# Damo12320/OptixPathtracer

Hardware: AMD Instinct MI355X
Metric: Msamples/sec at 1920x1080, max-depth 8; MSE vs reference (higher is better)
Workload: dtype f32; 1 GPU; BASELINE configs[1]: Diffuse sphere-in-box 1920x1080, 1024 spp, depth 8, 1xMI355X; scene=sphere_box_diffuse, triangles=34570, width=1920, height=1080, max_depth=8, material_mode=lambert, kernel=auto (wavefront), frames_per_launch=128, wavefront_streams=1, parallelism=spp-shard x1, batch_frames=128, queue_bytes=55207544320, queue_budget_bytes=77305217024, bvh_builder=auto (GPU binned SAH + GPU SAH-optimal BVH4 collapse), primary_dedup=True

## Files before the change

### include/ptamd.h

```cpp
#ifndef PTAMD_H
#define PTAMD_H
#include <stddef.h>
#include <stdint.h>

#ifdef __cplusplus
extern "C" {
#endif

#define PT_OK 0
#define PT_ERR_INVALID (-1)
#define PT_ERR_HIP (-2)
#define PT_ERR_STATE (-3)
#define PT_ERR_NOMEM (-4)

#define PT_MAT_DEFAULT 0
#define PT_MAT_LAMBERT 1
#define PT_MAT_CONDUCTOR 2
#define PT_MAT_DIELECTRIC 3
#define PT_MAT_LAYERED 4

#define PT_KERNEL_MEGA 0
#define PT_KERNEL_WAVEFRONT 1
#define PT_BVH_AUTO 0
#define PT_BVH_LBVH 1
// ... 85 lines not shown
    uint64_t pair_kernel_launches;
    uint64_t pair_kernel_rays;
    uint64_t pair_kernel_bytes;
    uint64_t pair_kernel_shadow_rays;
    uint64_t nee_unoccluded;
    uint64_t queue_bytes;
    uint64_t queue_budget;
    int32_t last_streams;
    int32_t last_batch_frames;
    uint64_t look_ahead_held;
    uint64_t lit_table_answers;
    uint64_t lit_table_cells;
    uint64_t lit_table_bits_set;
    uint64_t lit_table_bytes;
    double lit_table_build_ms;
    uint64_t geometry_commits;
    uint64_t geometry_refits;
    uint64_t geometry_rebuilds;
    double geometry_commit_ms;
    double bvh_sah_cost;
    double bvh_sah_cost_built;
} pt_stats;

typedef struct pt_renderer pt_renderer;

int pt_create(const pt_scene* scene, const pt_options* options, pt_renderer** out);
int pt_destroy(pt_renderer* r);

int pt_resize(pt_renderer* r, int32_t width, int32_t height);
int pt_set_camera(pt_renderer* r, const float position[3], const float inverse_view[16],
// ... 11 lines not shown
int pt_set_primary_dedup(pt_renderer* r, int32_t enable);
int pt_set_wavefront_streams(pt_renderer* r, int32_t streams);
int pt_set_band_split(pt_renderer* r, int32_t enable);
int pt_set_lit_table(pt_renderer* r, int32_t enable);
typedef struct pt_lit_table_info {
    int32_t active;
    int32_t lights;
    uint32_t triangles;
    uint32_t cells;
    uint32_t words_per_light;
    float delta;
    float margin;
} pt_lit_table_info;
int pt_lit_table_download(pt_renderer* r, pt_lit_table_info* info, uint32_t* tri_words, int64_t tri_bytes,
                          uint32_t* bits, int64_t bits_bytes);

typedef struct pt_launch_params {
    struct {
        float* color_buffer;
        int32_t size[2];
        uint32_t id;
    } frame;
    struct {
        float position[3];
        float inverse_view_matrix[16];
        float inverse_projection_matrix[16];
    } camera;
    const pt_point_light* point_lights;
    int32_t point_light_count;
    int32_t max_bounces;
// ... 87 lines not shown
```

### optixpathtracer_amd/capi.py

```python
from __future__ import annotations

import ctypes as C
import os
from pathlib import Path

_HERE = Path(__file__).resolve().parent
LIB_PATH = _HERE / "libptamd.so"

PT_MAT_DEFAULT, PT_MAT_LAMBERT, PT_MAT_CONDUCTOR, PT_MAT_DIELECTRIC, PT_MAT_LAYERED = range(5)
PT_KERNEL_MEGA, PT_KERNEL_WAVEFRONT, PT_KERNEL_AUTO = 0, 1, 2
PT_BVH_AUTO, PT_BVH_LBVH, PT_BVH_SAH, PT_BVH_PLOC, PT_BVH_SAH_GPU = 0, 1, 2, 3, 4
PT_GEOM_REFIT, PT_GEOM_REBUILD = 0, 1
PT_OK, PT_ERR_INVALID, PT_ERR_HIP, PT_ERR_STATE, PT_ERR_NOMEM = 0, -1, -2, -3, -4

MATERIAL_MODES = {
    "default": PT_MAT_DEFAULT,
    "lambert": PT_MAT_LAMBERT,
    "conductor": PT_MAT_CONDUCTOR,
    "dielectric": PT_MAT_DIELECTRIC,
    "layered": PT_MAT_LAYERED,
}


class PTError(RuntimeError):
# ... 104 lines not shown
        ("pair_kernel_launches", C.c_uint64),
        ("pair_kernel_rays", C.c_uint64),
        ("pair_kernel_bytes", C.c_uint64),
        ("pair_kernel_shadow_rays", C.c_uint64),
        ("nee_unoccluded", C.c_uint64),
        ("queue_bytes", C.c_uint64),
        ("queue_budget", C.c_uint64),
        ("last_streams", C.c_int32),
        ("last_batch_frames", C.c_int32),
        ("look_ahead_held", C.c_uint64),
        ("lit_table_answers", C.c_uint64),
        ("lit_table_cells", C.c_uint64),
        ("lit_table_bits_set", C.c_uint64),
        ("lit_table_bytes", C.c_uint64),
        ("lit_table_build_ms", C.c_double),
        ("geometry_commits", C.c_uint64),
        ("geometry_refits", C.c_uint64),
        ("geometry_rebuilds", C.c_uint64),
        ("geometry_commit_ms", C.c_double),
        ("bvh_sah_cost", C.c_double),
        ("bvh_sah_cost_built", C.c_double),
    ]


class pt_lit_table_info(C.Structure):
    _fields_ = [("active", C.c_int32), ("lights", C.c_int32), ("triangles", C.c_uint32), ("cells", C.c_uint32),
                ("words_per_light", C.c_uint32), ("delta", C.c_float), ("margin", C.c_float)]


class _pt_launch_frame(C.Structure):
# ... 35 lines not shown
    "pt_set_queue_budget": (C.c_int, [_R, C.c_int64]),
    "pt_get_trace_coherence": (C.c_int, [_R, C.POINTER(C.c_uint64)]),
    "pt_set_debug_hold": (C.c_int, [_R, C.c_int32]),
    "pt_set_traversal_stats": (C.c_int, [_R, C.c_int32]),
    "pt_set_kernel_timing": (C.c_int, [_R, C.c_int32]),
    "pt_render": (C.c_int, [_R, _FP]),
    "pt_launch": (C.c_int, [_R, C.POINTER(pt_launch_params)]),
    "pt_accum_clear": (C.c_int, [_R]),
    "pt_render_frames": (C.c_int, [_R, C.c_uint32, C.c_uint32]),
    "pt_set_primary_dedup": (C.c_int, [_R, C.c_int32]),
    "pt_set_band_split": (C.c_int, [_R, C.c_int32]),
    "pt_set_wavefront_streams": (C.c_int, [_R, C.c_int32]),
    "pt_set_lit_table": (C.c_int, [_R, C.c_int32]),
    "pt_lit_table_download": (C.c_int, [_R, C.POINTER(pt_lit_table_info), C.c_void_p, C.c_int64, C.c_void_p,
                                        C.c_int64]),
    "pt_render_accumulate": (C.c_int, [_R, C.c_uint32, C.c_uint32, _FP]),
    "pt_set_accum_device_buffer": (C.c_int, [_R, C.c_void_p]),
    "pt_accum_device_ptr": (C.c_void_p, [_R]),
    "pt_accum_download": (C.c_int, [_R, _FP, C.c_float]),
    "pt_set_accum_fp64": (C.c_int, [_R, C.c_int32]),
    "pt_accum_device_ptr64": (C.c_void_p, [_R]),
    "pt_accum_download64": (C.c_int, [_R, C.POINTER(C.c_double)]),
    "pt_synchronize": (C.c_int, [_R]),
    "pt_stream": (C.c_void_p, [_R]),
    "pt_device_count": (C.c_int32, [_R]),
    "pt_devices": (C.c_int, [_R, C.POINTER(C.c_int32), C.c_int32]),
    "pt_frame_id": (C.c_uint32, [_R]),
    "pt_set_frame_id": (C.c_int, [_R, C.c_uint32]),
    "pt_get_stats": (C.c_int, [_R, C.POINTER(pt_stats)]),
    "pt_stats_reset": (C.c_int, [_R]),
# ... 64 lines not shown
```

### optixpathtracer_amd/csrc/pt_capi.cpp

```cpp
#include <hip/hip_runtime.h>
#include <rccl/rccl.h>

#include <algorithm>
#include <cmath>
#include <cstdio>
#include <cstdlib>
#include <cstring>
#include <string>
#include <vector>

#include "../../include/ptamd.h"
#include "pt_internal.h"
#include "pt_lit.h"

using namespace pt;

namespace {

thread_local std::string g_last_error;

int fail(int code, const std::string& msg) {
    g_last_error = msg;
    return code;
}
// ... 38 lines not shown
            e = hipEventElapsedTime(&ms, start[i], stop[i]);
            *ms_sum += ms;
        }
        used = 0;
        return e;
    }
    void destroy() {
        for (hipEvent_t e : start) (void)hipEventDestroy(e);
        for (hipEvent_t e : stop) (void)hipEventDestroy(e);
        start.clear();
        stop.clear();
        used = 0;
    }
};

constexpr int kCounters = 28;
constexpr size_t kMaxPendingEvents = 4096;
constexpr int kMinTraversalStack = std::min(stack_capacity(PT_WF_STACK), stack_capacity(PT_MK_STACK));

struct GeomHost {
    std::vector<float4> verts, norms;
    std::vector<int4> tidx;
    std::vector<float> model;
    std::vector<int> voff;
    std::vector<int> has_normals, alpha;
    std::vector<float4> uvs;
    int n_meshes() const { return (int)has_normals.size(); }
    int normal_mode(int m) const {
        if (!has_normals[(size_t)m]) return 0;
        const float* M = &model[16 * (size_t)m];
        for (int r = 0; r < 3; ++r) {
// ... 216 lines not shown
    int lit_mode = -1;
    uint32_t* d_lit_tri = nullptr;
    uint32_t* d_lit_bits = nullptr;
    uint32_t lit_cells = 0, lit_words = 0;
    uint32_t lit_words_cap = 0;
    float lit_diag = 0.0f;
    uint32_t lit_version = 1, lit_built_version = 0;
    const void* lit_built_lights = nullptr;
    int lit_built_n = 0;
    bool lit_active = false;
    bool lit_launch_call = false;
    hipEvent_t lit_ev[2] = {nullptr, nullptr};
    bool lit_ev_pending = false;
    double lit_build_ms = 0.0;
    int64_t lit_bits_set = -1;

    DevScene scene() const {
        DevScene S;
        S.nodes = d_nodes;
        S.isect = d_isect;
        S.shade = d_shade;
        S.mats = d_mats;
        S.tuv = d_tuv;
        S.texels = d_texels;
        S.texinfo = d_texinfo;
        S.ntri = ntri;
        S.n_nodes = bvh_nodes;
        S.lds_nodes = nullptr;
        S.n_lds = 0;
        return S;
// ... 47 lines not shown
    L.lights = r->d_lights;
    L.n_lights = r->n_lights;
    L.max_bounces = r->max_bounces;
    L.frame_base = frame_base;
    L.n_frames = n_frames;
    L.accum = accum;
    L.accum64 = accum64;
    L.frame_stride = frame_stride;
    L.counters = r->d_counters;
    L.debug_pixel = r->d_debug ? r->debug_pixel : -1;
    L.debug_frame = r->debug_frame;
    L.debug = r->d_debug;
    L.lit_tri = r->lit_active ? r->d_lit_tri : nullptr;
    L.lit_bits = r->d_lit_bits;
    L.lit_words = r->lit_words;
    return L;
}

#ifndef PT_LIT_TABLE
#define PT_LIT_TABLE 1
#endif
bool lit_wanted(const pt_renderer* r) {
    const bool pays = r->material_mode == PT_MAT_LAMBERT || r->material_mode == PT_MAT_DEFAULT ||
                      r->material_mode == PT_MAT_LAYERED;
    const bool on = r->lit_mode < 0 ? PT_LIT_TABLE != 0 && pays && !r->lit_launch_call : r->lit_mode > 0;
    return on && r->d_lit_tri && r->d_lights && r->n_lights >= 1 && r->n_lights <= kLitMaxLights;
}
int lit_prepare(pt_renderer* r) {
    r->lit_active = lit_wanted(r);
    if (!r->lit_active) return PT_OK;
    if (r->lit_built_version == r->lit_version && r->lit_built_lights == r->d_lights && r->lit_built_n == r->n_lights)
        return PT_OK;
    if (!r->lit_ev[0]) {
        PT_HIP(hipEventCreate(&r->lit_ev[0]), "hipEventCreate");
        PT_HIP(hipEventCreate(&r->lit_ev[1]), "hipEventCreate");
    }
    PT_HIP(hipEventRecord(r->lit_ev[0], r->stream), "hipEventRecord");
    PT_HIP(lit_build(r->scene(), r->d_lit_tri, r->lit_cells, r->lit_words, r->d_lights, r->n_lights, r->d_lit_bits,
                     r->lit_diag, r->stream),
           "lit_build");
    PT_HIP(hipEventRecord(r->lit_ev[1], r->stream), "hipEventRecord");
    r->lit_ev_pending = true;
    r->lit_bits_set = -1;
    r->lit_built_version = r->lit_version;
    r->lit_built_lights = r->d_lights;
    r->lit_built_n = r->n_lights;
    return PT_OK;
}

size_t queue_bytes_held(const pt_renderer* r) {
    size_t b = r->wf.paths > 0 ? wavefront_bytes(r->wf.paths, r->wf.max_bounces) : 0;
    for (int k = 1; k < pt_renderer::kMaxWFStreams; ++k)
        if (r->xwf[k].paths > 0) b += wavefront_bytes(r->xwf[k].paths, r->xwf[k].max_bounces);
    return b;
}

size_t queue_budget_bytes(const pt_renderer* r) {
    if (r->queue_budget < 0) return SIZE_MAX;
    if (r->queue_budget > 0) return (size_t)r->queue_budget;
    size_t total = 0;
    if (hipDeviceTotalMem(&total, r->device) != hipSuccess || total == 0) {
        (void)hipGetLastError();
// ... 567 lines not shown
        e = hipMalloc(&r->d_lit_bits, sizeof(uint32_t) * (size_t)words * kLitMaxLights);
        if (e == hipSuccess) r->lit_words_cap = words;
    }
    if (e == hipSuccess && !r->d_lit_tri) e = hipMalloc(&r->d_lit_tri, sizeof(uint32_t) * ntri);
    if (e == hipSuccess)
        e = hipMemcpy(r->d_lit_tri, lit_words_host.data(), sizeof(uint32_t) * ntri, hipMemcpyHostToDevice);
    if (e != hipSuccess) {
        if (r->d_lit_tri) (void)hipFree(r->d_lit_tri);
        r->d_lit_tri = nullptr;
        r->lit_cells = r->lit_words = 0;
        return hip_fail(e, "lit table");
    }
    r->lit_cells = cells;
    r->lit_words = words;
    r->lit_diag = diag;
    return PT_OK;
}

}

extern "C" {

const char* pt_last_error(void) { return g_last_error.c_str(); }
const char* pt_version(void) { return "ptamd 0.1.0 gfx950"; }

int pt_create(const pt_scene* scene, const pt_options* options, pt_renderer** out) {
    if (!out) return fail(PT_ERR_INVALID, "pt_create: out is NULL");
    *out = nullptr;
    if (!scene || scene->n_meshes < 0 || (scene->n_meshes > 0 && !scene->meshes))
        return fail(PT_ERR_INVALID, "pt_create: invalid scene");
// ... 230 lines not shown
    (void)hipSetDevice(r->device);
    if (r->d_part) (void)hipFree(r->d_part);
    if (r->d_part64) (void)hipFree(r->d_part64);
    if (r->d_accum64) (void)hipFree(r->d_accum64);
    (void)hipSetDevice(r->device);
    if (r->d_nodes) (void)hipFree(r->d_nodes);
    if (r->d_isect) (void)hipFree(r->d_isect);
    if (r->d_shade) (void)hipFree(r->d_shade);
    if (r->d_mats) (void)hipFree(r->d_mats);
    if (r->d_tuv) (void)hipFree(r->d_tuv);
    if (r->d_texels) (void)hipFree(r->d_texels);
    if (r->d_texinfo) (void)hipFree(r->d_texinfo);
    if (r->d_lights) (void)hipFree(r->d_lights);
    if (r->d_lit_tri) (void)hipFree(r->d_lit_tri);
    if (r->d_lit_bits) (void)hipFree(r->d_lit_bits);
    if (r->d_overts) (void)hipFree(r->d_overts);
    if (r->d_onorms) (void)hipFree(r->d_onorms);
    if (r->d_tidx) (void)hipFree(r->d_tidx);
    if (r->d_rmesh) (void)hipFree(r->d_rmesh);
    if (r->d_sah_part) (void)hipFree(r->d_sah_part);
    for (hipEvent_t e : r->geom_ev)
        if (e) (void)hipEventDestroy(e);
    for (hipEvent_t e : r->lit_ev)
        if (e) (void)hipEventDestroy(e);
    if (r->d_frame) (void)hipFree(r->d_frame);
    ring_free(r);
    if (r->d_accum) (void)hipFree(r->d_accum);
    if (r->d_display) (void)hipFree(r->d_display);
    if (r->d_counters) (void)hipFree(r->d_counters);
    if (r->d_debug) (void)hipFree(r->d_debug);
    if (r->d_cancel_seen) (void)hipFree(r->d_cancel_seen);
    if (r->h_cancel) (void)hipHostFree(r->h_cancel);
    if (r->h_hold_release) (void)hipHostFree(r->h_hold_release);
    wavefront_free(r->wf);
    for (int k = 1; k < pt_renderer::kMaxWFStreams; ++k) {
        wavefront_free(r->xwf[k]);
        if (r->xstream[k]) (void)hipStreamDestroy(r->xstream[k]);
        if (r->ev_join[k]) (void)hipEventDestroy(r->ev_join[k]);
// ... 571 lines not shown
        r->lit_built_n == r->n_lights) {
        const size_t nw = (size_t)r->lit_words * (size_t)r->lit_built_n;
        if (r->lit_bits_set < 0) {
            std::vector<uint32_t> hb(nw);
            PT_HIP(hipMemcpy(hb.data(), r->d_lit_bits, sizeof(uint32_t) * nw, hipMemcpyDeviceToHost),
                   "download lit table");
            int64_t n = 0;
            for (uint32_t w : hb) n += __builtin_popcount(w);
            r->lit_bits_set = n;
        }
        out->lit_table_cells = r->lit_cells;
        out->lit_table_bits_set = (uint64_t)r->lit_bits_set;
        out->lit_table_bytes = sizeof(uint32_t) * ((size_t)r->ntri + (size_t)r->lit_words * kLitMaxLights);
        out->lit_table_build_ms = r->lit_build_ms;
    }
    out->geometry_commits = r->geom_commits;
    out->geometry_refits = r->geom_refits;
    out->geometry_rebuilds = r->geom_rebuilds;
    out->geometry_commit_ms = r->geom_commit_ms;
    out->bvh_sah_cost = r->sah_cost;
    out->bvh_sah_cost_built = r->sah_cost_built;
    for (pt_renderer* p : r->peers) {
        pt_stats ps;
        rc = pt_get_stats(p, &ps);
        if (rc) return rc;
        out->segments += ps.segments;
        out->samples += ps.samples;
        out->nodes_visited += ps.nodes_visited;
        out->tri_tests += ps.tri_tests;
        out->rays += ps.rays;
// ... 2 lines not shown
        out->wave_active_lanes += ps.wave_active_lanes;
        out->wave_node_steps += ps.wave_node_steps;
        out->wave_tri_steps += ps.wave_tri_steps;
        out->wave_refills += ps.wave_refills;
        out->lds_nodes_visited += ps.lds_nodes_visited;
        out->shade_kernel_items += ps.shade_kernel_items;
        out->shadow_rays += ps.shadow_rays;
        out->trace_kernel_rays += ps.trace_kernel_rays;
        out->trace_kernel_bytes += ps.trace_kernel_bytes;
        out->strict_retraces += ps.strict_retraces;
        out->nee_unoccluded += ps.nee_unoccluded;
        out->pair_kernel_rays += ps.pair_kernel_rays;
        out->pair_kernel_bytes += ps.pair_kernel_bytes;
        out->pair_kernel_shadow_rays += ps.pair_kernel_shadow_rays;
        out->lit_table_answers += ps.lit_table_answers;
        out->queue_bytes += ps.queue_bytes;
    }
    return PT_OK;
}

int pt_stats_reset(pt_renderer* r) {
    if (!r) return fail(PT_ERR_INVALID, "pt_stats_reset: NULL");
    int rc = pt_synchronize(r);
    if (rc) return rc;
    for (pt_renderer* p : r->peers) {
        if ((rc = pt_stats_reset(p)) != PT_OK) return rc;
    }
    PT_HIP(hipSetDevice(r->device), "hipSetDevice");
    PT_HIP(hipMemset(r->d_counters, 0, kCounters * sizeof(unsigned long long)), "hipMemset counters");
    r->samples = 0;
// ... 301 lines not shown
    info->margin = lit_margin(r->lit_diag);
    PT_HIP(hipStreamSynchronize(r->stream), "hipStreamSynchronize");
    if (tri_words) {
        if (tri_bytes != (int64_t)(sizeof(uint32_t) * (size_t)r->ntri))
            return fail(PT_ERR_INVALID, "pt_lit_table_download: tri_words size mismatch");
        PT_HIP(hipMemcpy(tri_words, r->d_lit_tri, (size_t)tri_bytes, hipMemcpyDeviceToHost), "download lit table");
    }
    if (bits) {
        if (bits_bytes != (int64_t)(sizeof(uint32_t) * (size_t)r->lit_words * (size_t)r->n_lights))
            return fail(PT_ERR_INVALID, "pt_lit_table_download: bits size mismatch");
        PT_HIP(hipMemcpy(bits, r->d_lit_bits, (size_t)bits_bytes, hipMemcpyDeviceToHost), "download lit table");
    }
    return PT_OK;
}

extern "C" int pt_set_band_split(pt_renderer* r, int32_t enable) {
    if (!r) return fail(PT_ERR_INVALID, "pt_set_band_split: NULL");
    int rc = collect_pending(r);
    if (rc) return rc;
    r->band_split = enable != 0;
    for (pt_renderer* p : r->peers) {
        if ((rc = pt_set_band_split(p, enable)) != PT_OK) return rc;
    }
    return PT_OK;
}

extern "C" int pt_set_kernel_timing(pt_renderer* r, int32_t enable) {
    if (!r) return fail(PT_ERR_INVALID, "pt_set_kernel_timing: NULL");
    int rc = collect_pending(r);
    if (rc) return rc;
// ... 7 lines not shown
```

### optixpathtracer_amd/csrc/pt_device.h

```cpp
#pragma once
#include "pt_bsdf.h"

namespace pt {

constexpr int kEmptyChild = (int)0x80000000;

struct __align__(16) BNode4 {
    float4 lox, hix, loy, hiy, loz, hiz;
    int4 child;
    int4 pad;
};

__device__ __forceinline__ int leaf_first(int c) { return (~c) >> 3; }
__device__ __forceinline__ int leaf_count(int c) { return ((~c) & 7) + 1; }

struct DevScene {
    const BNode4* nodes;
    const float4* isect;
    const float4* shade;
    const float4* mats;
    const float4* tuv;
    const uint32_t* texels;
    const int4* texinfo;
    int ntri;
// ... 19 lines not shown
    const DevLight* lights;
    int n_lights;
    int max_bounces;
    uint32_t frame_base;
    uint32_t n_frames;
    float* accum;
    double* accum64;
    size_t frame_stride;
    unsigned long long* counters;
    int debug_pixel;
    uint32_t debug_frame;
    float* debug;
    const uint32_t* lit_tri;
    const uint32_t* lit_bits;
    uint32_t lit_words;
};
constexpr int kDebugMaxBounces = 64;
constexpr int kDebugRecordFloats = 22;

__device__ __forceinline__ int debug_path_id(const DevLaunch& L) {
    const uint32_t f = L.debug_frame - L.frame_base;
    const int P = L.width * L.height, p = L.debug_pixel - L.width * L.row0;
    return (L.debug_pixel >= 0 && p >= 0 && p < P && f < L.n_frames) ? (int)f * P + p : -1;
}

struct Hit {
    float t, u, v;
    int tri;
    int orig;
    bool back;
// ... 758 lines not shown
```

### optixpathtracer_amd/csrc/pt_internal.h

```cpp
#pragma once
#include <hip/hip_runtime.h>

#include <algorithm>
#include <vector>

#include "pt_device.h"

namespace pt {

struct BuildInput {
    const float4* tri_orig;
    const float4* nrm_orig;
    const float4* uv_orig;
    int n;
    float cmin[3], cmax[3];
    int builder;
    const float4* tri_host;
};
constexpr int kBuilderPLOC = 0;
constexpr int kBuilderLBVH = 1;
constexpr int kBuilderSAH = 2;
constexpr int kBuilderSAHGPU = 3;

void sah_binary_tree(const float4* tri, int n, std::vector<uint32_t>& order, std::vector<int2>& child,
// ... 53 lines not shown
hipError_t launch_wavefront_frame(int mode, bool stats, const DevScene& S, const DevLaunch& L, const WFState& W,
                                  uint32_t frame, int nf, bool primary_dedup, int cus, hipStream_t stream,
                                  const hipEvent_t* trace_events,
                                  int* n_timed = nullptr, hipEvent_t accum_wait = nullptr,
                                  hipEvent_t accum_done = nullptr, const hipEvent_t* shade_events = nullptr,
                                  int* n_shade_timed = nullptr, bool wide_trace = false);

hipError_t launch_render(int kernel, int mode, bool stats, const DevScene& S, const DevLaunch& L,
                         hipStream_t stream);
hipError_t launch_trace(const DevScene& S, const float* d_rays, int n, int* d_prim, float* d_thit, float* d_u,
                        float* d_v, int* d_back, int any_hit, hipStream_t stream);

bool lit_subdivide(const float4* isect, int ntri, std::vector<uint32_t>& words, uint32_t* cells, float* diagonal);
hipError_t lit_build(const DevScene& S, const uint32_t* tri_words, uint32_t cells, uint32_t words,
                     const DevLight* lights, int n_lights, uint32_t* bits, float diag, hipStream_t stream);

struct RefitMesh {
    float m[16];
    int dirty;
    int normal_mode;
    int pad[2];
};
hipError_t refit_rebake(const RefitMesh* meshes, const float4* overts, const float4* onorms, const int4* tidx, int n,
                        float4* isect, float4* shade, hipStream_t stream);
hipError_t refit_levels(BNode4* nodes, const float4* isect, const std::vector<int>& level_base, hipStream_t stream);
int sah_partial_blocks(int n_nodes);
hipError_t sah_partial_launch(const BNode4* nodes, int n_nodes, double* partial, hipStream_t stream);

hipError_t display_fill(float* p, size_t n, float v, hipStream_t stream);
hipError_t display_blend(float* fb, const float* frame, size_t n, float w, bool continuous, hipStream_t stream);
// ... 3 lines not shown
```

### optixpathtracer_amd/csrc/pt_lit.hip

```cpp
#include "pt_internal.h"
#include "pt_lit.h"

namespace pt {

bool lit_subdivide(const float4* isect, int ntri, std::vector<uint32_t>& words, uint32_t* cells, float* diagonal) {
    words.clear();
    *cells = 0;
    *diagonal = 0.0f;
    if (ntri <= 0) return false;
    float lo[3] = {INFINITY, INFINITY, INFINITY}, hi[3] = {-INFINITY, -INFINITY, -INFINITY};
    for (int t = 0; t < ntri; ++t) {
        const float4 A = isect[3 * t], E1 = isect[3 * t + 1], E2 = isect[3 * t + 2];
        const float v[3][3] = {{A.x, A.y, A.z}, {A.x + E1.x, A.y + E1.y, A.z + E1.z}, {A.x + E2.x, A.y + E2.y, A.z + E2.z}};
        for (int k = 0; k < 3; ++k)
            for (int a = 0; a < 3; ++a) {
                if (!(fabsf(v[k][a]) <= kLitMaxCoord)) return false;
                lo[a] = std::min(lo[a], v[k][a]);
                hi[a] = std::max(hi[a], v[k][a]);
            }
    }
    const double dx = (double)hi[0] - lo[0], dy = (double)hi[1] - lo[1], dz = (double)hi[2] - lo[2];
    const float diag = (float)std::sqrt(dx * dx + dy * dy + dz * dz);
    if (!(diag > 0.0f)) return false;
    const float target = kLitCellFraction * diag;
// ... 72 lines not shown
        } else {
            const int first = leaf_first(c), cnt = leaf_count(c);
            for (int q = 0; q < cnt; ++q) {
                const int u = first + q;
                const float4 UA = S.isect[3 * u], U1 = S.isect[3 * u + 1], U2 = S.isect[3 * u + 2];
                const double pa[3] = {UA.x, UA.y, UA.z};
                const double pb[3] = {(double)UA.x + U1.x, (double)UA.y + U1.y, (double)UA.z + U1.z};
                const double pc[3] = {(double)UA.x + U2.x, (double)UA.y + U2.y, (double)UA.z + U2.z};
                if (!lit_tri_outside(P, pa, pb, pc)) return;
            }
        }
    }
    atomicOr(&bits[(size_t)li * words + (cell >> 5)], 1u << (cell & 31));
}

}

hipError_t lit_build(const DevScene& S, const uint32_t* tri_words, uint32_t cells, uint32_t words,
                     const DevLight* lights, int n_lights, uint32_t* bits, float diag, hipStream_t stream) {
    hipError_t e = hipMemsetAsync(bits, 0, sizeof(uint32_t) * (size_t)words * (size_t)n_lights, stream);
    if (e != hipSuccess || n_lights <= 0) return e;
    const uint64_t n = (uint64_t)cells * (uint64_t)n_lights;
    hipLaunchKernelGGL(k_lit_build, dim3((unsigned)((n + kLitBlock - 1) / kLitBlock)), dim3(kLitBlock), 0, stream, S,
                       tri_words, cells, words, lights, n_lights, bits, diag);
    return hipGetLastError();
}

}
```

### optixpathtracer_amd/csrc/pt_wavefront.hip

```cpp
#include <type_traits>
#include <unordered_map>

#include "pt_internal.h"
#include "pt_lit.h"

namespace pt {

namespace {

constexpr int kBlockWF = 256;
#ifndef PT_TRACE_BLOCK
#define PT_TRACE_BLOCK 256
#endif
constexpr int kBlockTrace = PT_TRACE_BLOCK;
constexpr int kStack = PT_WF_STACK;
#ifndef PT_LDS_NODES
#define PT_LDS_NODES 49
#endif
constexpr int kLdsNodes = PT_LDS_NODES;
#ifndef PT_TRACE_BLOCK_WIDE
#define PT_TRACE_BLOCK_WIDE 768
#endif
#ifndef PT_LDS_NODES_WIDE
#define PT_LDS_NODES_WIDE 150
// ... 635 lines not shown
    return next_bounce < max_bounces && length(beta) > 0.00001f;
}

__device__ __forceinline__ int lit_cell(const DevLaunch& L, const Hit& h) {
    const uint32_t w = L.lit_tri[h.tri];
    const int k = lit_level(w);
    return k == kLitNoCells ? -1 : (int)(lit_first(w) + lit_cell_index(k, h.u, h.v));
}
__device__ __forceinline__ bool lit_bit(const DevLaunch& L, int li, int cell) {
    return (L.lit_bits[(size_t)li * L.lit_words + ((uint32_t)cell >> 5)] >> (cell & 31)) & 1u;
}
__device__ __forceinline__ void lit_count_wave(bool answered, int* lds) {
    const unsigned long long m = __ballot(answered ? 1 : 0);
    if (lane_id() == 0) lds[threadIdx.x >> 6] = __popcll(m);
}
template <int WAVES>
__device__ __forceinline__ void lit_count_block(const DevLaunch& L, const int* lds) {
    if (threadIdx.x != 0 || !L.counters) return;
    int tot = 0;
    for (int w = 0; w < WAVES; ++w) tot += lds[w];
    if (tot > 0) atomicAdd(&L.counters[27], (unsigned long long)tot);
}

__device__ __forceinline__ int vis0_index(const DevLaunch& L, int path, int li) {
    const int P1 = L.width * L.height;
    return li * P1 + path % P1;
}

template <bool TEX>
__global__ __launch_bounds__(kBlockWF) void k_shadow0_setup(DevScene S, DevLaunch L, WFState W) {
    const int P1 = L.width * L.height;
    const int nl = L.n_lights;
    const int n = P1 * nl;
    if (wf_cancelled(W)) return;
    for (int k = blockIdx.x * blockDim.x + threadIdx.x; k < n; k += gridDim.x * blockDim.x) {
        const int li = k / P1, p = k - li * P1;
// ... 16 lines not shown
    if (blockIdx.x == 0 && threadIdx.x == 0) *cnt(W, 0, kShadowQ) = n;
}

template <int MODE, bool TEX, bool SHADE0>
__global__ __launch_bounds__(shf_block(MODE), shf_waves(MODE)) void k_shade_fused(DevScene S, DevLaunch L, WFState W, int b, int vis0) {
    constexpr bool shade0 = SHADE0;
    constexpr bool kBetaQ = MODE == kModeLambert;
    constexpr bool kShareOrigin = MODE == kModeLambert;
    constexpr int kBlock = shf_block(MODE), kWaves = kBlock / 64;
    const int n = *cnt(W, b, kQueue);
    const float4* rd = W.ray_d[b & 1];
    float4* no = W.ray_o[(b + 1) & 1];
    float4* nd = W.ray_d[(b + 1) & 1];
    __shared__ int lds_sh[kSortKeys * kWaves + kSortKeys + 1], lds_q[kSortKeys * kWaves + kSortKeys + 1];
    __shared__ int lds_lit[kWaves];
    const bool lit = !vis0 && L.lit_tri;
    if (blockIdx.x == 0 && threadIdx.x == 0 && L.counters) atomicAdd(&L.counters[15], (unsigned long long)n);
    if ((int)(blockIdx.x * kBlock) >= n) return;
    {
        const int i = (int)(blockIdx.x * kBlock + threadIdx.x);
        const bool valid = i < n && !wf_cancelled(W);
        bool emit_shadow = false, emit_next = false, lit_answer = false;
        f3 so, sdir, contrib, o, d, beta;
        uint32_t seed = 0;
        float stmax = 0.0f;
        int path = 0;
        int shadow_light = 0;
        const int P1 = L.width * L.height;
        float4 l0 = make_float4(0.0f, 0.0f, 0.0f, 0.0f);
        if (valid) {
            const float4 hv = ldqs(W.hit + i);
            const float4 c_q = shade0 ? make_float4(0.0f, 0.0f, 0.0f, 0.0f) : ldqs(rd + i);
            const float4 bv_q = (!shade0 && kBetaQ) ? ldqs(queue_beta(W, b) + i) : make_float4(0.0f, 0.0f, 0.0f, 0.0f);
            path = __float_as_int(hv.x);
            const Hit h = decode_hit(hv);
            if (h.tri >= 0) {
                const int lit_c = lit ? lit_cell(L, h) : -1;
                const float4 c = shade0 ? ldqs(rd + path % P1) : c_q;
                d = mk(c.x, c.y, c.z);
                SurfaceHit sf;
                reconstruct<TEX>(S, h, d, sf);
                if (shade0) {
// ... 25 lines not shown
                        f3 Li = mk(lt.cr, lt.cg, lt.cb) / d2;
                        contrib = ((beta * spectrum) * Li) / (P * 1.0f);
                        lit_answer = lit_c >= 0 && dot(ldir, sf.ng) > kLitDelta && lit_bit(L, li, lit_c);
                        if (vis0 || lit_answer) {
                            if (lit_answer || W.vis[vis0_index(L, path, li)]) {
                                const float4 l = shade0 ? l0 : W.L[path];
                                l0 = make_float4(l.x + contrib.x, l.y + contrib.y, l.z + contrib.z, 0.0f);
                                if (!shade0) W.L[path] = l0;
                            }
                        } else {
                            so = sf.pos + 1e-3f * sf.ng;
                            sdir = normalize(ldir);
                            stmax = length(ldir);
                            emit_shadow = true;
                            shadow_light = li;
                        }
                    }
                }
                BSample bs;
                if (b + 1 < L.max_bounces &&
                    bsdf_sample<MODE>(seed, sf.albedo, sf.roughness, conductor, sf.wo, bs)) {
                    emit_next = continue_path(sf, bs, beta, o, d, b + 1, L.max_bounces);
                    if (!kBetaQ) stqs(W.beta + path, make_float4(beta.x, beta.y, beta.z, __uint_as_float(seed)));
                }
            }
        }
        if (shade0 && valid) W.L[path] = l0;
        if (lit) lit_count_wave(lit_answer, lds_lit);
        const int qi = PT_SORT_EXT ? block_append_sorted<kWaves, kSortKeys>(cnt(W, b + 1, kQueue), emit_next ? octant(d) : -1, lds_q)
                                   : block_append<kWaves>(cnt(W, b + 1, kQueue), emit_next, lds_q);
        if (lit) lit_count_block<kWaves>(L, lds_lit);
        if (emit_next) {
            stqs(no + qi, make_float4(o.x, o.y, o.z, __int_as_float(path)));
            stqs(nd + qi, make_float4(d.x, d.y, d.z, 0.0f));
            if (kBetaQ) stqs(queue_beta(W, b + 1) + qi, make_float4(beta.x, beta.y, beta.z, __uint_as_float(seed)));
        }
        const int si = PT_SORT_SHADOW ? block_append_sorted<kWaves, kSortKeys>(cnt(W, b, kShadowQ),
                                                                              emit_shadow ? (shadow_light & (kSortKeys - 1)) : -1, lds_sh)
                                      : block_append<kWaves>(cnt(W, b, kShadowQ), emit_shadow, lds_sh);
        if (emit_shadow) {
            const bool share = kShareOrigin && emit_next;
            if (!share) stqs(W.sh_o + si, make_float4(so.x, so.y, so.z, __int_as_float(path)));
            stqs(W.sh_d + si, make_float4(sdir.x, sdir.y, sdir.z, stmax));
            stqs(W.sh_c + si, make_float4(contrib.x, contrib.y, contrib.z, __int_as_float(share ? qi : -1)));
        }
    }
}

template <int MODE, bool TEX>
__global__ __launch_bounds__(shf_block(MODE), 1) void k_shade0_pixel(DevScene S, DevLaunch L, WFState W, int nf) {
    constexpr bool kBetaQ = MODE == kModeLambert;
    constexpr int kBlock = shf_block(MODE), kWaves = kBlock / 64;
    const int P1 = L.width * L.height;
    __shared__ int lds_q[kSortKeys * kWaves + kSortKeys + 1];
// ... 155 lines not shown
        atomicAdd(&counters[6], (unsigned long long)(n_ext + n_sh));
        atomicAdd(&counters[7], 48ull * (unsigned long long)(n_ext + n_sh));
        atomicAdd(&counters[16], (unsigned long long)(n_ext + n_sh));
        atomicAdd(&counters[17], 48ull * (unsigned long long)(n_ext + n_sh));
        atomicAdd(&counters[19], (unsigned long long)n_sh);
    }
    flush_trav_stats<STATS>(counters, ts);
}

template <int MODE, bool TEX>
__global__ __launch_bounds__(kBlockShA) void k_shade_a(DevScene S, DevLaunch L, WFState W, int b, int vis0) {
    const int n = *cnt(W, b, kQueue);
    const float4* rd = W.ray_d[b & 1];
    __shared__ int lds_sh[kWavesShA + 1];
    __shared__ int lds_nee[kNeeBuckets * (kWavesShA + 1)], lds_smp[kSmpBuckets * (kWavesShA + 1)];
    __shared__ int lds_lit[kWavesShA];
    const bool lit = !vis0 && L.lit_tri;
    if ((int)(blockIdx.x * kBlockShA) >= n) return;
    const int i = (int)(blockIdx.x * kBlockShA + threadIdx.x);
    bool emit = false, lit_answer = false;
    int nee_bucket = -1, smp_bucket = -1, code = 0;
    f3 so, sdir;
    float stmax = 0.0f;
    if (i < n && !wf_cancelled(W)) {
        const float4 hv = W.hit[i];
        const float4 c = rd[i];
        const int path = __float_as_int(hv.x);
        const Hit h = decode_hit(hv);
        if (h.tri >= 0) {
            const int lit_c = lit ? lit_cell(L, h) : -1;
            SurfaceHit sf;
            reconstruct<TEX>(S, h, mk(c.x, c.y, c.z), sf);
            float4 bv = W.beta[path];
            uint32_t seed = __float_as_uint(bv.w);
            if (path == debug_path_id(L)) {
// ... 18 lines not shown
                f3 ldir = mk(lt.px, lt.py, lt.pz) - sf.pos;
                const f3 ln = normalize(ldir);
                int nb = 0;
                if (MODE == kModeLayered || !conductor)
                    nb = PT_NEE_CROSS && !same_hemisphere(sf.wo, to_local(sf.fr, ln)) ? kNeeCross
                                                                                     : nee_layered_bucket(bk, sf.albedo);
                lit_answer = lit_c >= 0 && dot(ldir, sf.ng) > kLitDelta && lit_bit(L, li, lit_c);
                if (vis0 || lit_answer) {
                    if (lit_answer || W.vis[vis0_index(L, path, li)]) nee_bucket = nb;
                } else {
                    so = sf.pos + 1e-3f * sf.ng;
                    sdir = ln;
                    stmax = length(ldir);
                    code = i | (nb << kItemBits);
                    emit = true;
                }
            }
        }
    }
    if (lit) lit_count_wave(lit_answer, lds_lit);
    const int si = block_append<kWavesShA>(cnt(W, b, kShadowQ), emit, lds_sh);
    if (lit) lit_count_block<kWavesShA>(L, lds_lit);
    if (emit) {
        W.sh_o[si] = make_float4(so.x, so.y, so.z, __int_as_float(code));
        W.sh_d[si] = make_float4(sdir.x, sdir.y, sdir.z, stmax);
    }
    const int ni = block_append_k<kWavesShA, kNeeBuckets>(cnt(W, b, kNee0), nee_bucket, lds_nee);
    if (nee_bucket >= 0) W.nq[nee_index(W, nee_bucket, ni)] = i;
    const int mi = block_append_k<kWavesShA, kSmpBuckets>(cnt(W, b, kSmp0), smp_bucket, lds_smp);
    if (smp_bucket >= 0) W.sq[smp_index(W, smp_bucket, mi)] = i;
}

template <bool TEX, int BLK = kBlockTrace>
__global__ __launch_bounds__(BLK, wf_waves(false)) void k_shadow_vis(DevScene S, WFState W, int b, int table,
                                                                      unsigned long long* counters) {
    const int n = *cnt(W, b, kShadowQ);
    if (blockIdx.x == 0 && threadIdx.x == 0 && counters) atomicAdd(&counters[5], (unsigned long long)n);
// ... 580 lines not shown
```

### optixpathtracer_amd/renderer.py

```python
from __future__ import annotations

import ctypes as C
import dataclasses

import numpy as np

from . import capi
from .capi import check, fptr, load
from .scenes import Scene


def _f32(a, shape=None) -> np.ndarray:
    a = np.ascontiguousarray(a, dtype=np.float32)
    if shape is not None:
        a = a.reshape(shape)
    return a


class _SceneBinding:

    def __init__(self, scene: Scene):
        self.keep = []
        meshes = (capi.pt_mesh * max(1, len(scene.meshes)))()
        for i, m in enumerate(scene.meshes):
# ... 222 lines not shown
    def set_lit_table(self, enable: bool | None) -> None:
        check(self.lib.pt_set_lit_table(self.h, -1 if enable is None else (1 if enable else 0)), "pt_set_lit_table")

    def lit_table(self):
        info = capi.pt_lit_table_info()
        check(self.lib.pt_lit_table_download(self.h, C.byref(info), None, 0, None, 0), "pt_lit_table_download")
        d = {k: getattr(info, k) for k, _ in capi.pt_lit_table_info._fields_}
        if not info.active:
            return d, None, None
        tri = np.zeros(info.triangles, np.uint32)
        bits = np.zeros((info.lights, info.words_per_light), np.uint32)
        check(self.lib.pt_lit_table_download(self.h, C.byref(info), tri.ctypes.data, tri.nbytes, bits.ctypes.data,
                                             bits.nbytes), "pt_lit_table_download")
        return d, tri, bits

    def render_accumulate(self, spp: int, first_frame_id: int = 1) -> np.ndarray:
        w, h = self.size
        out = np.empty((h, w, 3), np.float32)
        check(self.lib.pt_render_accumulate(self.h, int(spp), int(first_frame_id), fptr(out)),
              "pt_render_accumulate")
        return out

    def set_accum_device_buffer(self, ptr: int | None) -> None:
        check(self.lib.pt_set_accum_device_buffer(self.h, C.c_void_p(ptr) if ptr else None),
              "pt_set_accum_device_buffer")

    def accum(self, scale: float = 1.0) -> np.ndarray:
        w, h = self.size
        out = np.empty((h, w, 3), np.float32)
        check(self.lib.pt_accum_download(self.h, fptr(out), float(scale)), "pt_accum_download")
# ... 94 lines not shown
```

Measured before the change: 1701 Msamples/sec.

## Add per-cell occluder table to resolve shadow rays with one triangle test

Builds a per-light, per-surface-cell table on the GPU. Each entry records the triangle hit by a ray from the cell centre toward the light. During shading, a shadow ray for an unlit cell first tests that cached triangle, and if it blocks the ray, no shadow ray is queued or traced through the BVH. This cuts shadow-queue traffic and any-hit traversal, at the cost of a build kernel, extra memory, a table lookup per shading point, and a possible stats-path download.

```diff
diff --git a/include/ptamd.h b/include/ptamd.h
--- a/include/ptamd.h
+++ b/include/ptamd.h
@@ -123,6 +123,10 @@
     uint64_t lit_table_bits_set;
     uint64_t lit_table_bytes;
     double lit_table_build_ms;
+    uint64_t occluder_table_bytes;
+    uint64_t occluder_table_candidates;
+    double occluder_table_build_ms;
+    uint64_t occluder_table_answers;
     uint64_t geometry_commits;
     uint64_t geometry_refits;
     uint64_t geometry_rebuilds;
@@ -164,6 +168,9 @@
 } pt_lit_table_info;
 int pt_lit_table_download(pt_renderer* r, pt_lit_table_info* info, uint32_t* tri_words, int64_t tri_bytes,
                           uint32_t* bits, int64_t bits_bytes);
+int pt_set_occluder_table(pt_renderer* r, int32_t enable);
+int pt_occluder_table_download(pt_renderer* r, int64_t* entries_out, int32_t* entries, int64_t bytes);
+int pt_occluder_table_upload(pt_renderer* r, const int32_t* entries, int64_t bytes);
 
 typedef struct pt_launch_params {
     struct {
diff --git a/optixpathtracer_amd/capi.py b/optixpathtracer_amd/capi.py
--- a/optixpathtracer_amd/capi.py
+++ b/optixpathtracer_amd/capi.py
@@ -142,6 +142,10 @@
         ("lit_table_bits_set", C.c_uint64),
         ("lit_table_bytes", C.c_uint64),
         ("lit_table_build_ms", C.c_double),
+        ("occluder_table_bytes", C.c_uint64),
+        ("occluder_table_candidates", C.c_uint64),
+        ("occluder_table_build_ms", C.c_double),
+        ("occluder_table_answers", C.c_uint64),
         ("geometry_commits", C.c_uint64),
         ("geometry_refits", C.c_uint64),
         ("geometry_rebuilds", C.c_uint64),
@@ -207,6 +211,9 @@
     "pt_set_lit_table": (C.c_int, [_R, C.c_int32]),
     "pt_lit_table_download": (C.c_int, [_R, C.POINTER(pt_lit_table_info), C.c_void_p, C.c_int64, C.c_void_p,
                                         C.c_int64]),
+    "pt_set_occluder_table": (C.c_int, [_R, C.c_int32]),
+    "pt_occluder_table_download": (C.c_int, [_R, C.POINTER(C.c_int64), C.c_void_p, C.c_int64]),
+    "pt_occluder_table_upload": (C.c_int, [_R, C.c_void_p, C.c_int64]),
     "pt_render_accumulate": (C.c_int, [_R, C.c_uint32, C.c_uint32, _FP]),
     "pt_set_accum_device_buffer": (C.c_int, [_R, C.c_void_p]),
     "pt_accum_device_ptr": (C.c_void_p, [_R]),
diff --git a/optixpathtracer_amd/csrc/pt_capi.cpp b/optixpathtracer_amd/csrc/pt_capi.cpp
--- a/optixpathtracer_amd/csrc/pt_capi.cpp
+++ b/optixpathtracer_amd/csrc/pt_capi.cpp
@@ -76,7 +76,7 @@
     }
 };
 
-constexpr int kCounters = 28;
+constexpr int kCounters = 29;
 constexpr size_t kMaxPendingEvents = 4096;
 constexpr int kMinTraversalStack = std::min(stack_capacity(PT_WF_STACK), stack_capacity(PT_MK_STACK));
 
@@ -323,6 +323,18 @@
     bool lit_ev_pending = false;
     double lit_build_ms = 0.0;
     int64_t lit_bits_set = -1;
+    int occ_mode = -1;
+    int* d_occ = nullptr;
+    size_t occ_cap = 0;
+    bool occ_alloc_failed = false;
+    uint32_t occ_built_version = 0;
+    const void* occ_built_lights = nullptr;
+    int occ_built_n = 0;
+    bool occ_active = false;
+    hipEvent_t occ_ev[2] = {nullptr, nullptr};
+    bool occ_ev_pending = false;
+    double occ_build_ms = 0.0;
+    int64_t occ_candidates = -1;
 
     DevScene scene() const {
         DevScene S;
@@ -400,6 +412,8 @@
     L.lit_tri = r->lit_active ? r->d_lit_tri : nullptr;
     L.lit_bits = r->d_lit_bits;
     L.lit_words = r->lit_words;
+    L.occ_tab = r->lit_active && r->occ_active ? r->d_occ : nullptr;
+    L.lit_cells = r->lit_cells;
     return L;
 }
 
@@ -412,11 +426,57 @@
     const bool on = r->lit_mode < 0 ? PT_LIT_TABLE != 0 && pays && !r->lit_launch_call : r->lit_mode > 0;
     return on && r->d_lit_tri && r->d_lights && r->n_lights >= 1 && r->n_lights <= kLitMaxLights;
 }
+#ifndef PT_OCC_TABLE
+#define PT_OCC_TABLE 1
+#endif
+bool occ_wanted(const pt_renderer* r) {
+    const bool has_code = r->material_mode == PT_MAT_LAMBERT || r->material_mode == PT_MAT_DEFAULT ||
+                          r->material_mode == PT_MAT_LAYERED;
+    const bool pays = has_code;
+    const bool on = r->occ_mode < 0 ? PT_OCC_TABLE != 0 && pays && r->lit_mode < 0 : r->occ_mode > 0;
+    return on && has_code && !r->occ_alloc_failed && lit_wanted(r);
+}
+int occ_prepare(pt_renderer* r) {
+    r->occ_active = occ_wanted(r);
+    if (!r->occ_active) return PT_OK;
+    if (r->occ_built_version == r->lit_version && r->occ_built_lights == r->d_lights && r->occ_built_n == r->n_lights)
+        return PT_OK;
+    const size_t need = (size_t)r->lit_cells * (size_t)r->n_lights;
+    if (need > r->occ_cap) {
+        if (r->d_occ) (void)hipFree(r->d_occ);
+        r->d_occ = nullptr;
+        r->occ_cap = 0;
+        if (hipMalloc(&r->d_occ, sizeof(int) * need) != hipSuccess) {
+            (void)hipGetLastError();
+            r->d_occ = nullptr;
+            r->occ_alloc_failed = true;
+            r->occ_active = false;
+            return PT_OK;
+        }
+        r->occ_cap = need;
+    }
+    if (!r->occ_ev[0]) {
+        PT_HIP(hipEventCreate(&r->occ_ev[0]), "hipEventCreate");
+        PT_HIP(hipEventCreate(&r->occ_ev[1]), "hipEventCreate");
+    }
+    PT_HIP(hipEventRecord(r->occ_ev[0], r->stream), "hipEventRecord");
+    PT_HIP(occ_build(r->scene(), r->d_lit_tri, r->lit_cells, r->lit_words, r->d_lights, r->n_lights, r->d_lit_bits,
+                     r->d_occ, r->stream),
+           "occ_build");
+    PT_HIP(hipEventRecord(r->occ_ev[1], r->stream), "hipEventRecord");
+    r->occ_ev_pending = true;
+    r->occ_candidates = -1;
+    r->occ_built_version = r->lit_version;
+    r->occ_built_lights = r->d_lights;
+    r->occ_built_n = r->n_lights;
+    return PT_OK;
+}
 int lit_prepare(pt_renderer* r) {
     r->lit_active = lit_wanted(r);
+    r->occ_active = false;
     if (!r->lit_active) return PT_OK;
     if (r->lit_built_version == r->lit_version && r->lit_built_lights == r->d_lights && r->lit_built_n == r->n_lights)
-        return PT_OK;
+        return occ_prepare(r);
     if (!r->lit_ev[0]) {
         PT_HIP(hipEventCreate(&r->lit_ev[0]), "hipEventCreate");
         PT_HIP(hipEventCreate(&r->lit_ev[1]), "hipEventCreate");
@@ -431,7 +491,7 @@
     r->lit_built_version = r->lit_version;
     r->lit_built_lights = r->d_lights;
     r->lit_built_n = r->n_lights;
-    return PT_OK;
+    return occ_prepare(r);
 }
 
 size_t queue_bytes_held(const pt_renderer* r) {
@@ -1029,6 +1089,7 @@
     r->lit_cells = cells;
     r->lit_words = words;
     r->lit_diag = diag;
+    r->occ_alloc_failed = false;
     return PT_OK;
 }
 
@@ -1289,6 +1350,7 @@
     if (r->d_lights) (void)hipFree(r->d_lights);
     if (r->d_lit_tri) (void)hipFree(r->d_lit_tri);
     if (r->d_lit_bits) (void)hipFree(r->d_lit_bits);
+    if (r->d_occ) (void)hipFree(r->d_occ);
     if (r->d_overts) (void)hipFree(r->d_overts);
     if (r->d_onorms) (void)hipFree(r->d_onorms);
     if (r->d_tidx) (void)hipFree(r->d_tidx);
@@ -1297,6 +1359,8 @@
     for (hipEvent_t e : r->geom_ev)
         if (e) (void)hipEventDestroy(e);
     for (hipEvent_t e : r->lit_ev)
+        if (e) (void)hipEventDestroy(e);
+    for (hipEvent_t e : r->occ_ev)
         if (e) (void)hipEventDestroy(e);
     if (r->d_frame) (void)hipFree(r->d_frame);
     ring_free(r);
@@ -1898,6 +1962,29 @@
         out->lit_table_bytes = sizeof(uint32_t) * ((size_t)r->ntri + (size_t)r->lit_words * kLitMaxLights);
         out->lit_table_build_ms = r->lit_build_ms;
     }
+    out->occluder_table_answers = c[28];
+    if (r->occ_ev_pending) {
+        float ms = 0.0f;
+        if (hipEventElapsedTime(&ms, r->occ_ev[0], r->occ_ev[1]) == hipSuccess)
+            r->occ_build_ms = ms;
+        else
+            (void)hipGetLastError();
+        r->occ_ev_pending = false;
+    }
+    if (occ_wanted(r) && r->d_occ && r->occ_built_version == r->lit_version && r->occ_built_lights == r->d_lights &&
+        r->occ_built_n == r->n_lights) {
+        const size_t ne = (size_t)r->lit_cells * (size_t)r->occ_built_n;
+        if (r->occ_candidates < 0) {
+            std::vector<int> ho(ne);
+            PT_HIP(hipMemcpy(ho.data(), r->d_occ, sizeof(int) * ne, hipMemcpyDeviceToHost), "download occluder table");
+            int64_t n = 0;
+            for (int t : ho) n += t >= 0;
+            r->occ_candidates = n;
+        }
+        out->occluder_table_bytes = sizeof(int) * ne;
+        out->occluder_table_candidates = (uint64_t)r->occ_candidates;
+        out->occluder_table_build_ms = r->occ_build_ms;
+    }
     out->geometry_commits = r->geom_commits;
     out->geometry_refits = r->geom_refits;
     out->geometry_rebuilds = r->geom_rebuilds;
@@ -1930,6 +2017,7 @@
         out->pair_kernel_bytes += ps.pair_kernel_bytes;
         out->pair_kernel_shadow_rays += ps.pair_kernel_shadow_rays;
         out->lit_table_answers += ps.lit_table_answers;
+        out->occluder_table_answers += ps.occluder_table_answers;
         out->queue_bytes += ps.queue_bytes;
     }
     return PT_OK;
@@ -2261,6 +2349,49 @@
     return PT_OK;
 }
 
+extern "C" int pt_set_occluder_table(pt_renderer* r, int32_t enable) {
+    if (!r) return fail(PT_ERR_INVALID, "pt_set_occluder_table: NULL");
+    const int mode = enable < 0 ? -1 : (enable > 0 ? 1 : 0);
+    r->occ_mode = mode;
+    for (pt_renderer* p : r->peers) p->occ_mode = mode;
+    return PT_OK;
+}
+
+extern "C" int pt_occluder_table_download(pt_renderer* r, int64_t* entries_out, int32_t* entries, int64_t bytes) {
+    if (!r || !entries_out) return fail(PT_ERR_INVALID, "pt_occluder_table_download: NULL");
+    PT_HIP(hipSetDevice(r->device), "hipSetDevice");
+    int rc = lit_prepare(r);
+    if (rc) return rc;
+    *entries_out = r->occ_active ? (int64_t)r->lit_cells * (int64_t)r->n_lights : 0;
+    if (!r->occ_active || !entries) return PT_OK;
+    if (bytes != (int64_t)sizeof(int32_t) * *entries_out)
+        return fail(PT_ERR_INVALID, "pt_occluder_table_download: size mismatch");
+    PT_HIP(hipStreamSynchronize(r->stream), "hipStreamSynchronize");
+    PT_HIP(hipMemcpy(entries, r->d_occ, (size_t)bytes, hipMemcpyDeviceToHost), "download occluder table");
+    return PT_OK;
+}
+
+extern "C" int pt_occluder_table_upload(pt_renderer* r, const int32_t* entries, int64_t bytes) {
+    if (!r || !entries) return fail(PT_ERR_INVALID, "pt_occluder_table_upload: NULL");
+    PT_HIP(hipSetDevice(r->device), "hipSetDevice");
+    int rc = pt_synchronize(r);
+    if (rc) return rc;
+    if ((rc = lit_prepare(r)) != PT_OK) return rc;
+    if (!r->occ_active) return fail(PT_ERR_INVALID, "pt_occluder_table_upload: the table is not in use");
+    const int64_t n = (int64_t)r->lit_cells * (int64_t)r->n_lights;
+    if (bytes != (int64_t)sizeof(int32_t) * n) return fail(PT_ERR_INVALID, "pt_occluder_table_upload: size mismatch");
+    for (int64_t i = 0; i < n; ++i)
+        if (entries[i] < -1 || entries[i] >= r->ntri)
+            return fail(PT_ERR_INVALID, "pt_occluder_table_upload: entry out of range");
+    PT_HIP(hipStreamSynchronize(r->stream), "hipStreamSynchronize");
+    PT_HIP(hipMemcpy(r->d_occ, entries, (size_t)bytes, hipMemcpyHostToDevice), "upload occluder table");
+    r->occ_candidates = -1;
+    for (pt_renderer* p : r->peers) {
+        if ((rc = pt_occluder_table_upload(p, entries, bytes)) != PT_OK) return rc;
+    }
+    return PT_OK;
+}
+
 extern "C" int pt_set_band_split(pt_renderer* r, int32_t enable) {
     if (!r) return fail(PT_ERR_INVALID, "pt_set_band_split: NULL");
     int rc = collect_pending(r);
diff --git a/optixpathtracer_amd/csrc/pt_device.h b/optixpathtracer_amd/csrc/pt_device.h
--- a/optixpathtracer_amd/csrc/pt_device.h
+++ b/optixpathtracer_amd/csrc/pt_device.h
@@ -57,6 +57,8 @@
     const uint32_t* lit_tri;
     const uint32_t* lit_bits;
     uint32_t lit_words;
+    const int* occ_tab;
+    uint32_t lit_cells;
 };
 constexpr int kDebugMaxBounces = 64;
 constexpr int kDebugRecordFloats = 22;
diff --git a/optixpathtracer_amd/csrc/pt_internal.h b/optixpathtracer_amd/csrc/pt_internal.h
--- a/optixpathtracer_amd/csrc/pt_internal.h
+++ b/optixpathtracer_amd/csrc/pt_internal.h
@@ -91,6 +91,8 @@
 bool lit_subdivide(const float4* isect, int ntri, std::vector<uint32_t>& words, uint32_t* cells, float* diagonal);
 hipError_t lit_build(const DevScene& S, const uint32_t* tri_words, uint32_t cells, uint32_t words,
                      const DevLight* lights, int n_lights, uint32_t* bits, float diag, hipStream_t stream);
+hipError_t occ_build(const DevScene& S, const uint32_t* tri_words, uint32_t cells, uint32_t words,
+                     const DevLight* lights, int n_lights, const uint32_t* bits, int* occ, hipStream_t stream);
 
 struct RefitMesh {
     float m[16];
diff --git a/optixpathtracer_amd/csrc/pt_lit.hip b/optixpathtracer_amd/csrc/pt_lit.hip
--- a/optixpathtracer_amd/csrc/pt_lit.hip
+++ b/optixpathtracer_amd/csrc/pt_lit.hip
@@ -110,6 +110,70 @@
     atomicOr(&bits[(size_t)li * words + (cell >> 5)], 1u << (cell & 31));
 }
 
+constexpr int kOccStack = 2 * kSpillDepth + 2;
+static_assert(kOccStack / 2 > kSpillDepth && kOccStack - 3 > 72, "k_occ_build: the spill must stay unused");
+
+__global__ __launch_bounds__(kLitBlock) void k_occ_build(DevScene S, const uint32_t* __restrict__ tri_words,
+                                                        uint32_t cells, uint32_t words, const DevLight* __restrict__ lights,
+                                                        int n_lights, const uint32_t* __restrict__ bits,
+                                                        int* __restrict__ occ) {
+    __shared__ int lds_stack[kOccStack * kLitBlock];
+    __shared__ int lds_spill[1];
+    const uint64_t id = (uint64_t)blockIdx.x * kLitBlock + threadIdx.x;
+    if (id >= (uint64_t)cells * (uint64_t)n_lights) return;
+    const int li = (int)(id / cells);
+    const uint32_t cell = (uint32_t)(id - (uint64_t)li * cells);
+    int cand = -1;
+    do {
+        if ((bits[(size_t)li * words + (cell >> 5)] >> (cell & 31)) & 1u) break;
+        int a = 0, b = S.ntri - 1;
+        while (a < b) {
+            const int m = (a + b + 1) >> 1;
+            if (lit_first(tri_words[m]) <= cell) a = m; else b = m - 1;
+        }
+        const int t = a;
+        const uint32_t w = tri_words[t];
+        const int k = lit_level(w);
+        if (k == kLitNoCells || cell - lit_first(w) >= lit_cells(k)) break;
+        const DevLight lt = lights[li];
+        if (!(fabsf(lt.px) <= kLitMaxCoord && fabsf(lt.py) <= kLitMaxCoord && fabsf(lt.pz) <= kLitMaxCoord)) break;
+        const float4 A = S.isect[3 * t], E1 = S.isect[3 * t + 1], E2 = S.isect[3 * t + 2];
+        int cu[3], cv[3];
+        lit_cell_corners(k, cell - lit_first(w), cu, cv);
+        const float s = 1.0f / (3.0f * (float)(1 << k));
+        const float u = (float)(cu[0] + cu[1] + cu[2]) * s, v = (float)(cv[0] + cv[1] + cv[2]) * s;
+        const f3 e1 = mk(E1.x, E1.y, E1.z), e2 = mk(E2.x, E2.y, E2.z);
+        const f3 p = mk(A.x, A.y, A.z) + u * e1 + v * e2;
+        const f3 n = cross(e1, e2);
+        const float nl = length(n);
+        if (!(nl > 0.0f)) break;
+        f3 ng = n / nl;
+        const f3 ldir = mk(lt.px, lt.py, lt.pz) - p;
+        float h = dot(ldir, ng);
+        if (h < 0.0f) {
+            ng = -ng;
+            h = -h;
+        }
+        if (!(h > kLitDelta)) break;
+        TravState st;
+        TravStats ts;
+        trav_init(st, p + 1e-3f * ng, normalize(ldir), 0.0f, length(ldir));
+        while (!trav_step<kRayClosest, false, kOccStack, false>(S, st, lds_stack + threadIdx.x, kLitBlock, lds_spill, ts)) {
+        }
+        if (st.h.tri >= 0 && st.h.tri < S.ntri && __float_as_int(S.isect[3 * st.h.tri + 2].w) == 0) cand = st.h.tri;
+    } while (false);
+    occ[id] = cand;
+}
+
+}
+
+hipError_t occ_build(const DevScene& S, const uint32_t* tri_words, uint32_t cells, uint32_t words,
+                     const DevLight* lights, int n_lights, const uint32_t* bits, int* occ, hipStream_t stream) {
+    if (n_lights <= 0 || cells == 0) return hipSuccess;
+    const uint64_t n = (uint64_t)cells * (uint64_t)n_lights;
+    hipLaunchKernelGGL(k_occ_build, dim3((unsigned)((n + kLitBlock - 1) / kLitBlock)), dim3(kLitBlock), 0, stream, S,
+                       tri_words, cells, words, lights, n_lights, bits, occ);
+    return hipGetLastError();
 }
 
 hipError_t lit_build(const DevScene& S, const uint32_t* tri_words, uint32_t cells, uint32_t words,
diff --git a/optixpathtracer_amd/csrc/pt_wavefront.hip b/optixpathtracer_amd/csrc/pt_wavefront.hip
--- a/optixpathtracer_amd/csrc/pt_wavefront.hip
+++ b/optixpathtracer_amd/csrc/pt_wavefront.hip
@@ -673,12 +673,24 @@
     const unsigned long long m = __ballot(answered ? 1 : 0);
     if (lane_id() == 0) lds[threadIdx.x >> 6] = __popcll(m);
 }
-template <int WAVES>
+template <int WAVES, int SLOT = 27>
 __device__ __forceinline__ void lit_count_block(const DevLaunch& L, const int* lds) {
     if (threadIdx.x != 0 || !L.counters) return;
     int tot = 0;
     for (int w = 0; w < WAVES; ++w) tot += lds[w];
-    if (tot > 0) atomicAdd(&L.counters[27], (unsigned long long)tot);
+    if (tot > 0) atomicAdd(&L.counters[SLOT], (unsigned long long)tot);
+}
+constexpr int kOccCounter = 28;
+template <bool TEX>
+__device__ __forceinline__ bool occ_answers(const DevScene& S, int t, f3 o, f3 d, float tmax) {
+    if (t < 0) return false;
+    const float4 A = S.isect[3 * t], E1 = S.isect[3 * t + 1], E2 = S.isect[3 * t + 2];
+    float th, uh, vh;
+    bool bk;
+    if (!tri_test(A, E1, E2, o, d, 0.0f, tmax, th, uh, vh, bk)) return false;
+    if (TEX && __float_as_int(E2.w) != 0) return false;
+    const f3 inv = safe_inv(d);
+    return tri_accept(A, E1, E2, inv, mk(o.x * inv.x, o.y * inv.y, o.z * inv.z), th);
 }
 
 __device__ __forceinline__ int vis0_index(const DevLaunch& L, int path, int li) {
@@ -725,7 +737,10 @@
     float4* nd = W.ray_d[(b + 1) & 1];
     __shared__ int lds_sh[kSortKeys * kWaves + kSortKeys + 1], lds_q[kSortKeys * kWaves + kSortKeys + 1];
     __shared__ int lds_lit[kWaves];
+    constexpr bool kOcc = MODE == kModeLambert;
+    __shared__ int lds_occ[kOcc ? kWaves : 1];
     const bool lit = !vis0 && L.lit_tri;
+    const bool occ = kOcc && lit && L.occ_tab;
     if (blockIdx.x == 0 && threadIdx.x == 0 && L.counters) atomicAdd(&L.counters[15], (unsigned long long)n);
     if ((int)(blockIdx.x * kBlock) >= n) return;
     {
@@ -737,6 +752,7 @@
         float stmax = 0.0f;
         int path = 0;
         int shadow_light = 0;
+        int occ_t = -1;
         const int P1 = L.width * L.height;
         float4 l0 = make_float4(0.0f, 0.0f, 0.0f, 0.0f);
         if (valid) {
@@ -792,6 +808,8 @@
                             stmax = length(ldir);
                             emit_shadow = true;
                             shadow_light = li;
+                            if (kOcc && occ && lit_c >= 0 && dot(ldir, sf.ng) > kLitDelta)
+                                occ_t = L.occ_tab[li * (int)L.lit_cells + lit_c];
                         }
                     }
                 }
@@ -813,9 +831,20 @@
             stqs(nd + qi, make_float4(d.x, d.y, d.z, 0.0f));
             if (kBetaQ) stqs(queue_beta(W, b + 1) + qi, make_float4(beta.x, beta.y, beta.z, __uint_as_float(seed)));
         }
+        if constexpr (kOcc) {
+            if (occ) {
+                bool answered = false;
+                if (occ_t >= 0) answered = occ_answers<TEX>(S, occ_t, (kShareOrigin && emit_next) ? o : so, sdir, stmax);
+                if (answered) emit_shadow = false;
+                lit_count_wave(answered, lds_occ);
+            }
+        }
         const int si = PT_SORT_SHADOW ? block_append_sorted<kWaves, kSortKeys>(cnt(W, b, kShadowQ),
                                                                               emit_shadow ? (shadow_light & (kSortKeys - 1)) : -1, lds_sh)
                                       : block_append<kWaves>(cnt(W, b, kShadowQ), emit_shadow, lds_sh);
+        if constexpr (kOcc) {
+            if (occ) lit_count_block<kWaves, kOccCounter>(L, lds_occ);
+        }
         if (emit_shadow) {
             const bool share = kShareOrigin && emit_next;
             if (!share) stqs(W.sh_o + si, make_float4(so.x, so.y, so.z, __int_as_float(path)));
@@ -1001,11 +1030,12 @@
     const float4* rd = W.ray_d[b & 1];
     __shared__ int lds_sh[kWavesShA + 1];
     __shared__ int lds_nee[kNeeBuckets * (kWavesShA + 1)], lds_smp[kSmpBuckets * (kWavesShA + 1)];
-    __shared__ int lds_lit[kWavesShA];
+    __shared__ int lds_lit[kWavesShA], lds_occ[kWavesShA];
     const bool lit = !vis0 && L.lit_tri;
+    const bool occ = lit && L.occ_tab;
     if ((int)(blockIdx.x * kBlockShA) >= n) return;
     const int i = (int)(blockIdx.x * kBlockShA + threadIdx.x);
-    bool emit = false, lit_answer = false;
+    bool emit = false, lit_answer = false, occ_answer = false;
     int nee_bucket = -1, smp_bucket = -1, code = 0;
     f3 so, sdir;
     float stmax = 0.0f;
@@ -1054,13 +1084,18 @@
                     stmax = length(ldir);
                     code = i | (nb << kItemBits);
                     emit = true;
+                    if (occ && lit_c >= 0 && dot(ldir, sf.ng) > kLitDelta)
+                        occ_answer = occ_answers<TEX>(S, L.occ_tab[li * (int)L.lit_cells + lit_c], so, sdir, stmax);
+                    if (occ_answer) emit = false;
                 }
             }
         }
     }
     if (lit) lit_count_wave(lit_answer, lds_lit);
+    if (occ) lit_count_wave(occ_answer, lds_occ);
     const int si = block_append<kWavesShA>(cnt(W, b, kShadowQ), emit, lds_sh);
     if (lit) lit_count_block<kWavesShA>(L, lds_lit);
+    if (occ) lit_count_block<kWavesShA, kOccCounter>(L, lds_occ);
     if (emit) {
         W.sh_o[si] = make_float4(so.x, so.y, so.z, __int_as_float(code));
         W.sh_d[si] = make_float4(sdir.x, sdir.y, sdir.z, stmax);
diff --git a/optixpathtracer_amd/renderer.py b/optixpathtracer_amd/renderer.py
--- a/optixpathtracer_amd/renderer.py
+++ b/optixpathtracer_amd/renderer.py
@@ -260,6 +260,23 @@
                                              bits.nbytes), "pt_lit_table_download")
         return d, tri, bits
 
+    def set_occluder_table(self, enable: bool | None) -> None:
+        check(self.lib.pt_set_occluder_table(self.h, -1 if enable is None else (1 if enable else 0)),
+              "pt_set_occluder_table")
+
+    def occluder_table(self):
+        n = C.c_int64(0)
+        check(self.lib.pt_occluder_table_download(self.h, C.byref(n), None, 0), "pt_occluder_table_download")
+        if n.value == 0:
+            return None
+        e = np.zeros(n.value, np.int32)
+        check(self.lib.pt_occluder_table_download(self.h, C.byref(n), e.ctypes.data, e.nbytes), "pt_occluder_table_download")
+        return e
+
+    def upload_occluder_table(self, entries) -> None:
+        e = np.ascontiguousarray(entries, np.int32)
+        check(self.lib.pt_occluder_table_upload(self.h, e.ctypes.data, e.nbytes), "pt_occluder_table_upload")
+
     def render_accumulate(self, spp: int, first_frame_id: int = 1) -> np.ndarray:
         w, h = self.size
         out = np.empty((h, w, 3), np.float32)
```

New measurement: 1781 Msamples/sec, median of 6. 4.7% higher.
